# chao1224/GeoSSL

Measured on AMD Instinct MI355X. Metric: molecules/s/GPU SchNet+DDM fwd+bwd (QM9-sized, bs=1024); % HBM roofline, higher is better.
Workload: dtype f32

## Files before the change

### geossl_amd/csrc/ncsn_bwd.hip

```cpp
#include "common.h"
#include "geossl_hip.h"
#include "split.h"
#include "tn.h"

using namespace geossl;

namespace {

constexpr int TR = 32;

#ifdef NB_TIMING
__device__ long long nb_dbg[2 * 32 * 8];
#define NB_MARK(slot)                                                                              \
  do {                                                                                             \
    if (blockIdx.x == 5 && lane == 0 && (wave == 0 || wave == NW) && t - t_begin < 32)             \
      nb_dbg[((wave == 0 ? 0 : 1) * 32 + (t - t_begin)) * 8 + (slot)] = clock64();                 \
  } while (0)
#else
#define NB_MARK(slot) do {} while (0)
#endif

template <int NW>
struct NbLds {
  static constexpr int F = 32 * NW, H = F / 2, KHS = (H + 15) / 16, HMB = (H + 31) / 32, KS = F / 16;
  u32x4* zb;
  u32x4* dz2T;
  u32x4* fT;
  u32x4* dz1r;
  u32x4* abT;
  int4* scal;
  float* pdv;
  float* dep;
  float* wls;
  int* eg;
  int* ef;
  int* ea;
  int* ec;
  __device__ explicit NbLds(uint8_t* smem) {
    zb = reinterpret_cast<u32x4*>(smem);
    dz2T = zb + 2 * KHS * 2 * 64;
    fT = dz2T + HMB * 2 * 2 * 64;
    dz1r = fT + 2 * NW * 2 * 2 * 64;
    abT = dz1r + KS * 2 * 64;
    scal = reinterpret_cast<int4*>(abT + NW * 2 * 2 * 64);
    pdv = reinterpret_cast<float*>(scal + 3 * TR);
    dep = pdv + 3 * TR;
    wls = dep + NW * TR;
    eg = reinterpret_cast<int*>(wls + F);
    ef = eg + 4;
    ea = ef + 2 * NW;
    ec = ea + NW;
  }
  static size_t bytes() {
    return (size_t)(2 * KHS * 2 + HMB * 4 + 2 * NW * 4 + KS * 2 + NW * 4) * 1024 + 3 * TR * sizeof(int4) +
           (size_t)(3 * TR + NW * TR + F) * sizeof(float) + (size_t)(4 + 4 * NW) * sizeof(int);
  }
};

struct NcsnFusedArgs {
  const float* h;
  const int64_t* sei0;
  const int64_t* sei1;
  int S;
  GeosslNcsnWeights w;
  GeosslNcsnSaved sv;
  const int64_t* divisor;
  float out_scale;
  const float* gout;
  float* dfeat;
  float* demb;
  float* grow;
  float* pw1;
  float* pd1;
  float* pb1;
  float* pw2;
  float* pb2;
  float* psm;
};

__device__ __forceinline__ float ldg_off(const float* base, uint32_t byte_off) {
  return *reinterpret_cast<const float*>(reinterpret_cast<const char*>(base) + byte_off);
}
__device__ __forceinline__ int crow4(int r, int k4) { return (r & 3) + 8 * (r >> 2) + k4; }
__device__ __forceinline__ int opaque(int v) {
  asm volatile("" : "+v"(v));
  return v;
}
__device__ __forceinline__ u32x4 pack8(const f32x16& t, int s) {
  u32x4 w;
#pragma unroll
  for (int q = 0; q < 4; ++q) {
    const f16x2 p = {(_Float16)t[8 * s + 2 * q], (_Float16)t[8 * s + 2 * q + 1]};
    w[q] = __builtin_bit_cast(uint32_t, p);
  }
  return w;
}
__device__ __forceinline__ const u32x4& piece(const Frag2& f, int pc) { return pc == 0 ? f.h : f.l; }
__device__ __forceinline__ int scale_exponent(float m) { return max(mag_exponent(m), -40); }
__device__ __forceinline__ float pow2(int e) { return __builtin_amdgcn_ldexpf(1.0f, e); }
constexpr int E_NONE = -100000;

template <int NW, bool ROLE_A>
__device__ __forceinline__ void ncsn_bwd_body(const NcsnFusedArgs& a, const int S, const float* __restrict__ a_h) {
  using L_t = NbLds<NW>;
  constexpr int F = L_t::F, H = L_t::H, KHS = L_t::KHS, HMB = L_t::HMB, KS = L_t::KS, NT = 128 * NW;
  extern __shared__ __attribute__((aligned(16))) uint8_t smem_raw[];
  const L_t L(smem_raw);
  const int tid = threadIdx.x, lane = tid & 63, j = lane & 31, kh = lane >> 5;
  const int wave = __builtin_amdgcn_readfirstlane(tid >> 6);
  const int nb = ROLE_A ? wave : wave - NW;
  const int ntiles = (S + TR - 1) / TR;
  const int per = (ntiles + (int)gridDim.x - 1) / (int)gridDim.x;
  const int t_begin = (int)blockIdx.x * per, t_end = min(ntiles, t_begin + per);
  const float scale = a.out_scale * (a.gout != nullptr ? a.gout[0] : 1.0f) / (float)a.divisor[0];
  const uint32_t col = 32 * nb + j;

  Frag2 wreg[ROLE_A ? KHS : KS];
  f32x16 accw1[ROLE_A ? NW : 1];
  f32x16 accw2[ROLE_A ? 1 : HMB];
  int E1[ROLE_A ? NW : 1];
  int E2 = E_NONE;
  int ew = 0;
  float bsum = 0.0f, dsum = 0.0f;
  u32x4 ident[2];
  float w3r[8];
  float s_w2 = 0.0f, s_w1 = 0.0f, s_b1 = 0.0f, s_g = 0.0f, s_d = 0.0f;
  float iw1 = 0.0f, ib1 = 0.0f, iw2 = 0.0f;
  int e3;
  {
    float m3 = 0.0f;
    for (int i = lane; i < H; i += 64) m3 = fmaxf(m3, fabsf(a.w.o3_w[i]));
    e3 = scale_exponent(wave_max(m3));
  }
  if constexpr (ROLE_A) {
    iw1 = a.w.in_w1[col];
    ib1 = a.w.in_b1[col];
    iw2 = a.w.in_w2[col];
    float raw[KHS][8];
    float wm = 0.0f, csum = 0.0f;
#pragma unroll
    for (int ks = 0; ks < KHS; ++ks)
#pragma unroll
      for (int e = 0; e < 8; ++e) {
        const int m = 16 * ks + 8 * kh + e;
        const float v = m < H ? a.w.o2_w[(size_t)m * F + col] : 0.0f;
        raw[ks][e] = v;
        wm = fmaxf(wm, fabsf(v));
        csum = fmaf(fabsf(v), m < H ? fabsf(a.w.o3_w[m]) : 0.0f, csum);
      }
    ew = scale_exponent(wave_max(wm));
    const float sw = pow2(14 - ew);
#pragma unroll
    for (int ks = 0; ks < KHS; ++ks) wreg[ks] = split8h_scaled(raw[ks], sw);
    csum += __shfl_xor(csum, 32, 64);
    const int ecw = max(mag_exponent(wave_max(csum)), -80);
    if (lane == 0) L.ec[nb] = ecw;
#pragma unroll
    for (int kb = 0; kb < NW; ++kb) {
      E1[kb] = E_NONE;
#pragma unroll
      for (int r = 0; r < 16; ++r) accw1[kb][r] = 0.0f;
    }
#pragma unroll
    for (int s = 0; s < 2; ++s)
#pragma unroll
      for (int q = 0; q < 4; ++q) {
        const int k0 = 16 * s + kperm(2 * q, kh), k1 = 16 * s + kperm(2 * q + 1, kh);
        ident[s][q] = (k0 == j ? 0x3C00u : 0u) | (k1 == j ? 0x3C000000u : 0u);
      }
  } else {
    float raw[KS][8];
    float wm = 0.0f;
#pragma unroll
    for (int ks = 0; ks < KS; ++ks)
#pragma unroll
      for (int e = 0; e < 8; ++e) {
        raw[ks][e] = a.w.o1_w[(size_t)(16 * ks + kperm(e, kh)) * (F + 1) + col];
        wm = fmaxf(wm, fabsf(raw[ks][e]));
      }
    ew = scale_exponent(wave_max(wm));
    const float sw = pow2(14 - ew);
#pragma unroll
    for (int ks = 0; ks < KS; ++ks) wreg[ks] = split8h_scaled(raw[ks], sw);
#pragma unroll
    for (int e = 0; e < 8; ++e) {
      const int m = 16 * nb + 8 * kh + e;
      w3r[e] = (nb < KHS && m < H) ? a.w.o3_w[m] : 0.0f;
    }
#pragma unroll
    for (int mb = 0; mb < HMB; ++mb)
#pragma unroll
      for (int r = 0; r < 16; ++r) accw2[mb][r] = 0.0f;
#pragma unroll
    for (int q2 = 0; q2 < 2; ++q2)
#pragma unroll
      for (int q = 0; q < 4; ++q) {
        const int k0 = 16 * q2 + 8 * kh + 2 * q;
        ident[q2][q] = (k0 == j ? 0x3C00u : 0u) | (k0 + 1 == j ? 0x3C000000u : 0u);
      }
  }
  for (int i = tid; i < F; i += NT) L.wls[i] = a.w.o1_w[(size_t)i * (F + 1) + F];

  int sc_u = 0, sc_v = 0;
  float sc_g = 0.0f, sc_e = 0.0f, sc_p = 0.0f;
  int EG = -60;
  auto load_scal = [&](int tt) {
    if constexpr (ROLE_A) {
      if (wave == 0) {
        const int row = min(TR * tt + j, S - 1);
        sc_u = (int)a.sei0[row];
        sc_v = (int)a.sei1[row];
        sc_g = a.sv.gscale[row];
        sc_e = a.sv.emb[row];
        sc_p = a.sv.pd[row];
      }
    }
  };
  auto put_scal = [&](int tt) {
    if constexpr (ROLE_A) {
      if (wave == 0) {
        const int row = TR * tt + lane;
        const bool valid = lane < TR && row < S && tt < t_end;
        const float gr = valid ? pin(sc_g) * scale : 0.0f;
        EG = max(EG, mag_exponent(wave_max(fabsf(gr))));
        if (lane < TR) {
          L.scal[(tt % 3) * TR + lane] = make_int4(sc_u, sc_v, __float_as_int(gr), __float_as_int(sc_e));
          L.pdv[(tt % 3) * TR + lane] = sc_p;
          if (valid) a.grow[row] = gr;
        }
        if (lane == 0) L.eg[tt % 3] = EG;
      }
    }
  };
  float a1raw[16];
  auto request_a1 = [&](int tt, int k4) {
    if constexpr (ROLE_A) {
#pragma unroll
      for (int r = 0; r < 16; ++r)
        a1raw[r] = ldg_off(a.sv.a1, ((uint32_t)min(TR * tt + crow4(r, k4), S - 1) * (uint32_t)F + col) * 4u);
    }
  };
  f32x4 a2raw[2];
  float o3acc[8] = {0.0f, 0.0f, 0.0f, 0.0f, 0.0f, 0.0f, 0.0f, 0.0f};
  auto request_a2 = [&](int tt) {
    if constexpr (!ROLE_A) {
      if (nb < KHS) {
        const uint32_t off = ((uint32_t)min(TR * tt + j, S - 1) * (uint32_t)H + (16 * nb + 8 * kh)) * 4u;
        a2raw[0] = *reinterpret_cast<const f32x4*>(reinterpret_cast<const char*>(a.sv.a2) + off);
        a2raw[1] = *reinterpret_cast<const f32x4*>(reinterpret_cast<const char*>(a.sv.a2) + 16 + off);
      }
    }
  };
  float hu[16], hv[16];
  auto request_gather = [&](int tt, int k4) {
    if constexpr (!ROLE_A) {
      const int2* sc = reinterpret_cast<const int2*>(L.scal + (tt % 3) * TR);
#pragma unroll
      for (int r = 0; r < 16; ++r) {
        const int2 uv = sc[2 * crow4(r, k4)];
        hu[r] = ldg_off(a_h, ((uint32_t)uv.x * (uint32_t)F + col) * 4u);
        hv[r] = ldg_off(a_h, ((uint32_t)uv.y * (uint32_t)F + col) * 4u);
      }
    }
  };
  auto build_zb = [&](int tt) {
    if constexpr (!ROLE_A) {
      if (nb < KHS) {
        const float gr = __int_as_float(L.scal[(tt % 3) * TR + j].z);
        const float sz = pow2(14 - e3 - __builtin_amdgcn_readfirstlane(L.eg[tt % 3]));
        const float av[8] = {a2raw[0].x, a2raw[0].y, a2raw[0].z, a2raw[0].w, a2raw[1].x, a2raw[1].y, a2raw[1].z, a2raw[1].w};
        float v[8];
#pragma unroll
        for (int e = 0; e < 8; ++e) {
          const float a2v = pin(av[e]);
          v[e] = a2v > 0.0f ? gr * w3r[e] : 0.0f;
          o3acc[e] = fmaf(gr, a2v, o3acc[e]);
        }
        const Frag2 f = split8h_scaled(v, sz);
        u32x4* dst = L.zb + (size_t)(((tt & 1) * KHS + nb) * 2) * 64 + lane;
        dst[0] = f.h;
        dst[64] = f.l;
      }
    }
  };
  int EF = -40;
  auto build_fT = [&](int tt) {
    if constexpr (!ROLE_A) {
      float v[16];
      float m = 0.0f;
#pragma unroll
      for (int r = 0; r < 16; ++r) {
        v[r] = pin(hu[r]) + pin(hv[r]);
        m = fmaxf(m, fabsf(v[r]));
      }
      EF = max(EF, mag_exponent(wave_max(m)));
      const float sf = pow2(14 - EF);
      if (lane == 0) L.ef[(tt & 1) * NW + nb] = EF;
#pragma unroll
      for (int s = 0; s < 2; ++s) {
        float vv[8];
#pragma unroll
        for (int e = 0; e < 8; ++e) vv[e] = v[8 * s + e];
        const Frag2 f = split8h_scaled(vv, sf);
        u32x4* dst = L.fT + (size_t)((((tt & 1) * NW + nb) * 2 + s) * 2) * 64 + lane;
        dst[0] = f.h;
        dst[64] = f.l;
      }
    }
  };

  load_scal(t_begin);
  put_scal(t_begin);
  load_scal(t_begin + 1);
  put_scal(t_begin + 1);
  load_scal(t_begin + 2);
  if (t_begin < t_end) {
    request_a1(t_begin, 4 * kh);
    request_a2(t_begin);
  }
  __syncthreads();
  int eC = -80;
#pragma unroll
  for (int i = 0; i < NW; ++i) eC = max(eC, __builtin_amdgcn_readfirstlane(L.ec[i]));
  if (t_begin < t_end) {
    request_gather(t_begin, 4 * kh);
    build_zb(t_begin);
    build_fT(t_begin);
    request_a2(t_begin + 1);
    request_gather(t_begin + 1, 4 * kh);
  }
  int EA = -40;
  const float kA = pow2(e3 + ew - eC - 14);
  for (int t = t_begin; t < t_end; ++t) {
    const int buf = t & 1;
    int k4 = opaque(4 * kh);
    NB_MARK(0);
    lds_barrier();
    NB_MARK(1);
    const int EGt = __builtin_amdgcn_readfirstlane(L.eg[t % 3]);
    if constexpr (ROLE_A) {
      put_scal(t + 2);
      const float kT = pow2(EGt + eC - 14);
      f32x16 acc0, acc1;
#pragma unroll
      for (int r = 0; r < 16; ++r) acc0[r] = acc1[r] = 0.0f;
      {
        const u32x4* zs = L.zb + (size_t)(buf * KHS * 2) * 64 + lane;
        Frag2 a0, an;
        a0.h = zs[0]; a0.l = zs[64];
#pragma unroll
        for (int ks = 0; ks < KHS; ++ks) {
          if (ks + 1 < KHS) {
            const u32x4* s0 = zs + (size_t)((ks + 1) * 2) * 64;
            an.h = s0[0]; an.l = s0[64];
          }
          __builtin_amdgcn_sched_barrier(0);
          mma3x2(acc0, acc1, a0, wreg[ks]);
          __builtin_amdgcn_sched_barrier(0);
          if (ks + 1 < KHS) a0 = an;
        }
      }
      NB_MARK(5);
      float v[16];
      {
        const int4* sc = L.scal + (t % 3) * TR;
        float tb = 0.0f, td = 0.0f, am = 0.0f;
#pragma unroll
        for (int r = 0; r < 16; ++r) {
          a1raw[r] = pin(a1raw[r]);
          v[r] = a1raw[r] > 0.0f ? (acc0[r] + acc1[r]) * kA : 0.0f;
          tb += v[r];
          td = fmaf(v[r], __int_as_float(sc[crow4(r, k4)].w), td);
          am = fmaxf(am, fabsf(a1raw[r]));
        }
        bsum = fmaf(tb, kT, bsum);
        dsum = fmaf(td, kT, dsum);
        EA = max(EA, mag_exponent(wave_max(am)));
      }
      {
        const float sa = pow2(14 - EA);
        if (lane == 0) L.ea[nb] = EA;
#pragma unroll
        for (int s = 0; s < 2; ++s) {
          float vv[8];
#pragma unroll
          for (int e = 0; e < 8; ++e) vv[e] = a1raw[8 * s + e];
          const Frag2 f = split8h_scaled(vv, sa);
          u32x4* dst = L.abT + (size_t)((nb * 2 + s) * 2) * 64 + lane;
          dst[0] = f.h;
          dst[64] = f.l;
        }
      }
      Frag2 da[2];
#pragma unroll
      for (int s = 0; s < 2; ++s) {
        float vv[8];
#pragma unroll
        for (int e = 0; e < 8; ++e) vv[e] = v[8 * s + e];
        da[s] = split8h(vv);
      }
      {
        float wl[16];
#pragma unroll
        for (int r = 0; r < 16; ++r) wl[r] = L.wls[32 * nb + crow4(r, k4)];
        float de = 0.0f;
#pragma unroll
        for (int pc = 1; pc >= 0; --pc) {
          f32x16 tp;
#pragma unroll
          for (int r = 0; r < 16; ++r) tp[r] = 0.0f;
          tp = mfma_f16(piece(da[0], pc), ident[0], tp);
          tp = mfma_f16(piece(da[1], pc), ident[1], tp);
#pragma unroll
          for (int r = 0; r < 16; ++r) de = fmaf(tp[r], wl[r], de);
#pragma unroll
          for (int half = 0; half < 2; ++half)
            L.dz1r[(size_t)((2 * nb + half) * 2 + pc) * 64 + lane] = pack8(tp, half);
        }
        de += __shfl_xor(de, 32, 64);
        if (kh == 0) L.dep[j * NW + nb] = de * kT;
      }
      NB_MARK(6);
#pragma unroll
      for (int kb = 0; kb < NW; ++kb) {
        const int En = EGt + __builtin_amdgcn_readfirstlane(L.ef[buf * NW + kb]);
        if (En != E1[kb]) {
          const float f = pow2(max(E1[kb] - En, -200));
#pragma unroll
          for (int r = 0; r < 16; ++r) accw1[kb][r] *= f;
          E1[kb] = En;
        }
#pragma unroll
        for (int s = 0; s < 2; ++s) {
          const u32x4* s0 = L.fT + (size_t)(((buf * NW + kb) * 2 + s) * 2) * 64 + lane;
          Frag2 bf;
          bf.h = s0[0]; bf.l = s0[64];
          mma3(accw1[kb], da[s], bf);
        }
      }
    } else {
      if (nb < HMB) {
        float tb = 0.0f;
#pragma unroll
        for (int pc = 1; pc >= 0; --pc) {
          f32x16 tp;
#pragma unroll
          for (int r = 0; r < 16; ++r) tp[r] = 0.0f;
#pragma unroll
          for (int q = 0; q < 2; ++q) {
            if (2 * nb + q < KHS) {
              const u32x4* s0 = L.zb + (size_t)((buf * KHS + 2 * nb + q) * 2 + pc) * 64 + lane;
              tp = mfma_f16(s0[0], ident[q], tp);
            }
          }
#pragma unroll
          for (int r = 0; r < 16; ++r) tb += tp[r];
#pragma unroll
          for (int s = 0; s < 2; ++s) L.dz2T[(size_t)((nb * 2 + s) * 2 + pc) * 64 + lane] = pack8(tp, s);
        }
        bsum = fmaf(tb, pow2(EGt + e3 - 14), bsum);
      }
      NB_MARK(5);
      build_zb(t + 1);
      NB_MARK(6);
      build_fT(t + 1);
    }
    k4 = opaque(4 * kh);
    NB_MARK(2);
    lds_barrier();
    NB_MARK(3);
    if constexpr (ROLE_A) {
      request_a1(t + 1, k4);
      load_scal(t + 3);
      {
        const int4* sc = L.scal + (t % 3) * TR;
        const float* pdr = L.pdv + (t % 3) * TR;
#pragma unroll
        for (int i = 0; i < 16; ++i) {
          const int rl = 4 * k4 + i;
          float de = 0.0f;
#pragma unroll
          for (int n2 = 0; n2 < NW; ++n2) de += L.dep[rl * NW + n2];
          const float pd = pdr[rl];
          const float pre = fmaf(iw1, pd, ib1);
          s_w2 = fmaf(de, fmaxf(pre, 0.0f), s_w2);
          const float dp = pre > 0.0f ? de * iw2 : 0.0f;
          s_w1 = fmaf(dp, pd, s_w1);
          s_b1 += dp;
          if (wave == 0 && j == i) {
            s_g += __int_as_float(sc[rl].z);
            s_d += de;
          }
        }
      }
    } else {
      request_a2(t + 2);
      request_gather(t + 2, k4);
      NB_MARK(7);
      f32x16 acc0, acc1;
#pragma unroll
      for (int r = 0; r < 16; ++r) acc0[r] = acc1[r] = 0.0f;
      {
        const u32x4* zs = L.dz1r + lane;
        Frag2 b0, bn;
        b0.h = zs[0]; b0.l = zs[64];
#pragma unroll
        for (int ks = 0; ks < KS; ++ks) {
          if (ks + 1 < KS) {
            const u32x4* s0 = zs + (size_t)((ks + 1) * 2) * 64;
            bn.h = s0[0]; bn.l = s0[64];
          }
          __builtin_amdgcn_sched_barrier(0);
          mma3x2(acc0, acc1, wreg[ks], b0);
          __builtin_amdgcn_sched_barrier(0);
          if (ks + 1 < KS) b0 = bn;
        }
      }
      const float kD = pow2(EGt + eC + ew - 28);
      f32x16 outp;
#pragma unroll
      for (int r = 0; r < 16; ++r) outp[r] = (acc0[r] + acc1[r]) * kD;
      const int row = TR * t + j;
      if (row < S) {
        const uint32_t off = ((uint32_t)row * (uint32_t)F + 32 * nb + 4 * kh) * 4u;
#pragma unroll
        for (int q = 0; q < 4; ++q)
          *reinterpret_cast<f32x4*>(reinterpret_cast<char*>(a.dfeat) + 32 * q + off) =
              f32x4{outp[4 * q], outp[4 * q + 1], outp[4 * q + 2], outp[4 * q + 3]};
        if (nb == 0 && kh == 0) {
          float de = 0.0f;
#pragma unroll
          for (int n2 = 0; n2 < NW; ++n2) de += L.dep[j * NW + n2];
          a.demb[row] = de;
        }
      }
      {
        const int En = EGt + __builtin_amdgcn_readfirstlane(L.ea[nb]);
        if (En != E2) {
          const float f = pow2(max(E2 - En, -200));
#pragma unroll
          for (int mb = 0; mb < HMB; ++mb)
#pragma unroll
            for (int r = 0; r < 16; ++r) accw2[mb][r] *= f;
          E2 = En;
        }
      }
#pragma unroll
      for (int s = 0; s < 2; ++s) {
        const u32x4* sb = L.abT + (size_t)((nb * 2 + s) * 2) * 64 + lane;
        Frag2 bf;
        bf.h = sb[0]; bf.l = sb[64];
#pragma unroll
        for (int mb = 0; mb < HMB; ++mb) {
          const u32x4* s0 = L.dz2T + (size_t)((mb * 2 + s) * 2) * 64 + lane;
          Frag2 af;
          af.h = s0[0]; af.l = s0[64];
          mma3(accw2[mb], af, bf);
        }
      }
    }
    NB_MARK(4);
  }
  const size_t pb = blockIdx.x;
  if constexpr (ROLE_A) {
    float* P1 = a.pw1 + pb * F * F;
#pragma unroll
    for (int kb = 0; kb < NW; ++kb) {
      const float f = pow2(max(E1[kb] + eC - 28, -200));
#pragma unroll
      for (int r = 0; r < 16; ++r) P1[(size_t)(32 * nb + c_row(r, lane)) * F + 32 * kb + j] = accw1[kb][r] * f;
    }
    const float sb = bsum + __shfl_xor(bsum, 32, 64), sd = dsum + __shfl_xor(dsum, 32, 64);
    if (kh == 0) {
      a.pb1[pb * F + col] = sb;
      a.pd1[pb * F + col] = sd;
    }
    float* Ps = a.psm + pb * (H + 3 * F + 2);
    const float t_w2 = s_w2 + __shfl_xor(s_w2, 32, 64);
    const float t_w1 = s_w1 + __shfl_xor(s_w1, 32, 64), t_b1 = s_b1 + __shfl_xor(s_b1, 32, 64);
    if (kh == 0) {
      Ps[H + col] = t_w2;
      Ps[H + F + col] = t_w1;
      Ps[H + 2 * F + col] = t_b1;
    }
    if (wave == 0) {
      const float tg = wave_sum(s_g), td = wave_sum(s_d);
      if (lane == 0) {
        Ps[H + 3 * F] = tg;
        Ps[H + 3 * F + 1] = td;
      }
    }
  } else {
    float* P2 = a.pw2 + pb * H * F;
    const float f = pow2(max(E2 + e3 - 28, -200));
#pragma unroll
    for (int mb = 0; mb < HMB; ++mb)
#pragma unroll
      for (int r = 0; r < 16; ++r) {
        const int m = 32 * mb + c_row(r, lane);
        if (m < H) P2[(size_t)m * F + col] = accw2[mb][r] * f;
      }
    const float sb = bsum + __shfl_xor(bsum, 32, 64);
    if (nb < HMB && kh == 0 && (int)col < H) a.pb2[pb * H + col] = sb;
    if (nb < KHS) {
      float* Ps = a.psm + pb * (H + 3 * F + 2);
#pragma unroll
      for (int e = 0; e < 8; ++e) {
        float v = o3acc[e];
#pragma unroll
        for (int o = 16; o > 0; o >>= 1) v += __shfl_xor(v, o, 64);
        const int m = 16 * nb + 8 * kh + e;
        if (j == 0 && m < H) Ps[m] = v;
      }
    }
  }
}

template <int NW>
__global__ __launch_bounds__(128 * NW) void k_ncsn_bwd_fused(NcsnFusedArgs a) {
  if ((int)(threadIdx.x >> 6) < NW) ncsn_bwd_body<NW, true>(a, a.S, a.h);
  else ncsn_bwd_body<NW, false>(a, a.S, a.h);
}
struct NcsnFusedPair { NcsnFusedArgs a[2]; };
template <int NW>
__global__ __launch_bounds__(128 * NW) void k_ncsn_bwd_fused2(NcsnFusedPair pr, const int32_t* __restrict__ dyn_S,
                                                              const int32_t* __restrict__ dyn_view) {
  const NcsnFusedArgs& a = pr.a[blockIdx.y];
  const int S = dyn_count(a.S, dyn_S);
  const float* h = a.h;
  if (dyn_view != nullptr && blockIdx.y == 1) h += (size_t)(*dyn_view) * (32 * NW);
  if ((int)(threadIdx.x >> 6) < NW) ncsn_bwd_body<NW, true>(a, S, h);
  else ncsn_bwd_body<NW, false>(a, S, h);
}

__device__ __forceinline__ void ncsn_reduce_all_block(const ReduceMulti& m, int nblk, int accumulate,
                                                      const float* __restrict__ psm, int F, const GeosslNcsnGrads& g,
                                                      float (*red)[64]) {
  const int mb = m.xoff[m.nseg];
  if ((int)blockIdx.x < mb) {
    reduce_multi_block(m, nblk, accumulate, red, 0);
    return;
  }
  const int H = F / 2, len = H + 3 * F + 2;
  const int i = ((int)blockIdx.x - mb) * 4 + (int)(threadIdx.x >> 6), lane = threadIdx.x & 63;
  if (i >= len) return;
  float s = 0.0f;
  for (int b = lane; b < nblk; b += 64) s += psm[(size_t)b * len + i];
  s = wave_sum(s);
  if (lane == 0) {
    float* dst;
    if (i < H) dst = g.o3_w + i;
    else if (i < H + F) dst = g.in_w2 + (i - H);
    else if (i < H + 2 * F) dst = g.in_w1 + (i - H - F);
    else if (i < H + 3 * F) dst = g.in_b1 + (i - H - 2 * F);
    else if (i == H + 3 * F) dst = g.o3_b;
    else dst = g.in_b2;
    *dst = accumulate ? *dst + s : s;
  }
}
__global__ __launch_bounds__(256) void k_ncsn_reduce_all(ReduceMulti m, int nblk, int accumulate,
                                                         const float* __restrict__ psm, int F, GeosslNcsnGrads g) {
  __shared__ float red[4][64];
  ncsn_reduce_all_block(m, nblk, accumulate, psm, F, g, red);
}
__global__ __launch_bounds__(256) void k_ncsn_reduce_all2(ReduceMulti m0, ReduceMulti m1, int nblk, int accumulate,
                                                          const float* __restrict__ psm0,
                                                          const float* __restrict__ psm1, int F, GeosslNcsnGrads g0,
                                                          GeosslNcsnGrads g1) {
  __shared__ float red[4][64];
  if (blockIdx.y == 0) ncsn_reduce_all_block(m0, nblk, accumulate, psm0, F, g0, red);
  else ncsn_reduce_all_block(m1, nblk, accumulate, psm1, F, g1, red);
}

inline int fused_blocks(int64_t S) {
  const int64_t ntiles = (S + TR - 1) / TR;
  return (int)(ntiles < 256 ? ntiles : 256);
}

}

#ifdef NB_TIMING
extern "C" int geossl_ncsn_bwd_debug_read(long long* host) {
  return (int)hipMemcpyFromSymbol(host, HIP_SYMBOL(nb_dbg), sizeof(long long) * 2 * 32 * 8);
}
#endif

extern "C" int64_t geossl_ddm_loss_bwd_fused_workspace_floats(int64_t S, int F) {
  const int64_t nb = fused_blocks(S), H = F / 2;
  return nb * ((int64_t)F * F + 2 * F + H * F + H + (H + 3 * F + 2));
}

extern "C" int geossl_ddm_loss_bwd_fused(const float* h, const int64_t* sei0, const int64_t* sei1, int64_t S, int64_t N,
                                         int F, const GeosslNcsnWeights* w, const GeosslNcsnSaved* saved,
                                         const int64_t* stats_divisor, float out_scale, const float* gout, float* dfeat,
                                         float* demb, float* grow, const GeosslNcsnGrads* grads, float* workspace,
                                         int accumulate, hipStream_t stream) {
  if (S <= 0) return 0;
  if (F != 32 && F != 64 && F != 128) return (int)hipErrorInvalidValue;
  if (S * (int64_t)F * 4 >= ((int64_t)1 << 32) || N * (int64_t)F * 4 >= ((int64_t)1 << 32)) return (int)hipErrorInvalidValue;
  const int nb = fused_blocks(S), H = F / 2;
  NcsnFusedArgs a;
  a.h = h; a.sei0 = sei0; a.sei1 = sei1; a.S = (int)S; a.w = *w; a.sv = *saved; a.divisor = stats_divisor;
  a.out_scale = out_scale; a.gout = gout; a.dfeat = dfeat; a.demb = demb; a.grow = grow;
  a.pw1 = workspace;
  a.pd1 = a.pw1 + (size_t)nb * F * F;
  a.pb1 = a.pd1 + (size_t)nb * F;
  a.pw2 = a.pb1 + (size_t)nb * F;
  a.pb2 = a.pw2 + (size_t)nb * H * F;
  a.psm = a.pb2 + (size_t)nb * H;
#define LAUNCH(NWV)                                                                                      \
  do {                                                                                                   \
    allow_big_lds(&k_ncsn_bwd_fused<NWV>);                                                               \
    hipLaunchKernelGGL((k_ncsn_bwd_fused<NWV>), dim3(nb), dim3(128 * NWV), NbLds<NWV>::bytes(), stream, a); \
  } while (0)
  if (F == 128) LAUNCH(4); else if (F == 64) LAUNCH(2); else LAUNCH(1);
#undef LAUNCH
  GEOSSL_CHECK_LAUNCH();
  ReduceMulti rm;
  float* o1w[1] = {grads->o1_w};
  float* o1c[1] = {grads->o1_w + F};
  float* o1b[1] = {grads->o1_b};
  float* o2w[1] = {grads->o2_w};
  float* o2b[1] = {grads->o2_b};
  rm.add(a.pw1, F * F, F, F + 1, 1, o1w, 1);
  rm.add(a.pd1, F, F, F, F + 1, o1c, 1);
  rm.add(a.pb1, F, F, F, 1, o1b, 1);
  rm.add(a.pw2, H * F, F, F, 1, o2w, 1);
  rm.add(a.pb2, H, H, H, 1, o2b, 1);
  hipLaunchKernelGGL(k_ncsn_reduce_all, dim3(rm.blocks() + (H + 3 * F + 2 + 3) / 4, 1), dim3(256), 0, stream, rm, nb,
                     accumulate, a.psm, F, *grads);
  GEOSSL_CHECK_LAUNCH();
  return 0;
}

namespace geossl {
int launch_incidence_gather2(const float* dfeat0, const float* dfeat1, const int64_t* inc_ptr, const int32_t* inc_idx,
                             int64_t N, int F, float* dh0, float* dh1, hipStream_t stream, const int32_t* dyn_view);
}

extern "C" int geossl_ddm_loss_bwd_fused2(const GeosslNcsnHeadBwd* heads, const int64_t* sei0, const int64_t* sei1,
                                          int64_t S, int64_t N, int F, const int64_t* stats_divisor, const float* gout,
                                          const int64_t* inc_ptr, const int32_t* inc_idx, int accumulate,
                                          hipStream_t stream) {
  return geossl_ddm_loss_bwd_fused2_dyn(heads, sei0, sei1, S, N, F, stats_divisor, gout, inc_ptr, inc_idx, accumulate,
                                        nullptr, nullptr, stream);
}

extern "C" int geossl_ddm_loss_bwd_fused2_dyn(const GeosslNcsnHeadBwd* heads, const int64_t* sei0, const int64_t* sei1,
                                              int64_t S, int64_t N, int F, const int64_t* stats_divisor,
                                              const float* gout, const int64_t* inc_ptr, const int32_t* inc_idx,
                                              int accumulate, const int32_t* dyn_S, const int32_t* dyn_view,
                                              hipStream_t stream) {
  if (S <= 0) return 0;
  if (heads == nullptr || (F != 32 && F != 64 && F != 128)) return (int)hipErrorInvalidValue;
  if (S * (int64_t)F * 4 >= ((int64_t)1 << 32) || N * (int64_t)F * 4 >= ((int64_t)1 << 32)) return (int)hipErrorInvalidValue;
  const int nb = (fused_blocks(S) + 1) / 2, H = F / 2;
  NcsnFusedPair pr;
  NcsnFusedArgs* a = pr.a;
  for (int k = 0; k < 2; ++k) {
    const GeosslNcsnHeadBwd& hd = heads[k];
    if (hd.h == nullptr || hd.dfeat == nullptr || hd.workspace == nullptr) return (int)hipErrorInvalidValue;
    NcsnFusedArgs& x = a[k];
    x.h = hd.h; x.sei0 = sei0; x.sei1 = sei1; x.S = (int)S; x.w = hd.w; x.sv = hd.saved; x.divisor = stats_divisor;
    x.out_scale = hd.out_scale; x.gout = gout; x.dfeat = hd.dfeat; x.demb = hd.demb; x.grow = hd.grow;
    x.pw1 = hd.workspace;
    x.pd1 = x.pw1 + (size_t)nb * F * F;
    x.pb1 = x.pd1 + (size_t)nb * F;
    x.pw2 = x.pb1 + (size_t)nb * F;
    x.pb2 = x.pw2 + (size_t)nb * H * F;
    x.psm = x.pb2 + (size_t)nb * H;
  }
#define LAUNCH2(NWV)                                                                                                \
  do {                                                                                                              \
    allow_big_lds(&k_ncsn_bwd_fused2<NWV>);                                                                         \
    hipLaunchKernelGGL((k_ncsn_bwd_fused2<NWV>), dim3(nb, 2), dim3(128 * NWV), NbLds<NWV>::bytes(), stream, pr,         \
                       dyn_S, dyn_view);                                                                            \
  } while (0)
  if (F == 128) LAUNCH2(4); else if (F == 64) LAUNCH2(2); else LAUNCH2(1);
#undef LAUNCH2
  GEOSSL_CHECK_LAUNCH();
  ReduceMulti rm[2];
  for (int k = 0; k < 2; ++k) {
    const GeosslNcsnGrads* grads = &heads[k].grads;
    float* o1w[1] = {grads->o1_w};
    float* o1c[1] = {grads->o1_w + F};
    float* o1b[1] = {grads->o1_b};
    float* o2w[1] = {grads->o2_w};
    float* o2b[1] = {grads->o2_b};
    rm[k].add(a[k].pw1, F * F, F, F + 1, 1, o1w, 1);
    rm[k].add(a[k].pd1, F, F, F, F + 1, o1c, 1);
    rm[k].add(a[k].pb1, F, F, F, 1, o1b, 1);
    rm[k].add(a[k].pw2, H * F, F, F, 1, o2w, 1);
    rm[k].add(a[k].pb2, H, H, H, 1, o2b, 1);
  }
  hipLaunchKernelGGL(k_ncsn_reduce_all2, dim3(rm[0].blocks() + (H + 3 * F + 2 + 3) / 4, 2), dim3(256), 0, stream, rm[0],
                     rm[1], nb, accumulate, a[0].psm, a[1].psm, F, heads[0].grads, heads[1].grads);
  GEOSSL_CHECK_LAUNCH();
  if (heads[0].dh != nullptr && heads[1].dh != nullptr)
    return launch_incidence_gather2(heads[0].dfeat, heads[1].dfeat, inc_ptr, inc_idx, N, F, heads[0].dh, heads[1].dh, stream,
                                    dyn_view);
  return 0;
}
```

Measured before the change: 430,100.

## Process two 32-row sub-tiles per barrier in fused NCSN backward kernel

Doubles the per-iteration row tile in the fused NCSN backward kernel to 64 rows, handled as two 32-row sub-tiles. Each LDS barrier now covers twice the work, and the a1/a2/gather prefetches are restructured around the sub-tiles. Several per-lane weight registers (o3_w, in_w1/b1/w2) move into LDS, and waves_per_eu(2) is added, both to ease register pressure. The old 32-row path stays available through an environment variable. The cost is more LDS per block, and the grid still uses the 32-row block count, so fewer tiles per block may hurt load balance.

```diff
diff --git a/geossl_amd/csrc/ncsn_bwd.hip b/geossl_amd/csrc/ncsn_bwd.hip
--- a/geossl_amd/csrc/ncsn_bwd.hip
+++ b/geossl_amd/csrc/ncsn_bwd.hip
@@ -19,10 +19,16 @@
 #else
 #define NB_MARK(slot) do {} while (0)
 #endif
-
-template <int NW>
+#ifdef NB_HALF_BARRIERS
+#define NB_TILE_BARRIER() do { if (((t - t_begin) & 1) == 0) lds_barrier(); } while (0)
+#else
+#define NB_TILE_BARRIER() lds_barrier()
+#endif
+
+template <int NW, int MB>
 struct NbLds {
   static constexpr int F = 32 * NW, H = F / 2, KHS = (H + 15) / 16, HMB = (H + 31) / 32, KS = F / 16;
+  static constexpr int TT = TR * MB, FB = MB == 1 ? 2 : 1;
   u32x4* zb;
   u32x4* dz2T;
   u32x4* fT;
@@ -32,28 +38,33 @@
   float* pdv;
   float* dep;
   float* wls;
+  float* w3s;
+  float* inw;
   int* eg;
   int* ef;
   int* ea;
   int* ec;
   __device__ explicit NbLds(uint8_t* smem) {
     zb = reinterpret_cast<u32x4*>(smem);
-    dz2T = zb + 2 * KHS * 2 * 64;
-    fT = dz2T + HMB * 2 * 2 * 64;
-    dz1r = fT + 2 * NW * 2 * 2 * 64;
-    abT = dz1r + KS * 2 * 64;
-    scal = reinterpret_cast<int4*>(abT + NW * 2 * 2 * 64);
-    pdv = reinterpret_cast<float*>(scal + 3 * TR);
-    dep = pdv + 3 * TR;
-    wls = dep + NW * TR;
-    eg = reinterpret_cast<int*>(wls + F);
-    ef = eg + 4;
-    ea = ef + 2 * NW;
-    ec = ea + NW;
+    dz2T = zb + 2 * MB * KHS * 2 * 64;
+    fT = dz2T + MB * HMB * 2 * 2 * 64;
+    dz1r = fT + FB * MB * NW * 2 * 2 * 64;
+    abT = dz1r + MB * KS * 2 * 64;
+    scal = reinterpret_cast<int4*>(abT + MB * NW * 2 * 2 * 64);
+    pdv = reinterpret_cast<float*>(scal + 3 * TT);
+    dep = pdv + 3 * TT;
+    wls = dep + NW * TT;
+    w3s = wls + F;
+    inw = w3s + 16 * KHS;
+    eg = reinterpret_cast<int*>(inw + 3 * F);
+    ef = eg + 8;
+    ea = ef + FB * MB * NW;
+    ec = ea + MB * NW;
   }
   static size_t bytes() {
-    return (size_t)(2 * KHS * 2 + HMB * 4 + 2 * NW * 4 + KS * 2 + NW * 4) * 1024 + 3 * TR * sizeof(int4) +
-           (size_t)(3 * TR + NW * TR + F) * sizeof(float) + (size_t)(4 + 4 * NW) * sizeof(int);
+    return (size_t)(MB * (2 * KHS * 2 + HMB * 4 + FB * NW * 4 + KS * 2 + NW * 4)) * 1024 + 3 * TT * sizeof(int4) +
+           (size_t)(3 * TT + NW * TT + F + 16 * KHS + 3 * F) * sizeof(float) +
+           (size_t)(8 + FB * MB * NW + MB * NW + NW) * sizeof(int);
   }
 };
 
@@ -76,6 +87,7 @@
   float* pw2;
   float* pb2;
   float* psm;
+  int tile32;
 };
 
 __device__ __forceinline__ float ldg_off(const float* base, uint32_t byte_off) {
@@ -100,16 +112,18 @@
 __device__ __forceinline__ float pow2(int e) { return __builtin_amdgcn_ldexpf(1.0f, e); }
 constexpr int E_NONE = -100000;
 
-template <int NW, bool ROLE_A>
+template <int NW, bool ROLE_A, int MB>
 __device__ __forceinline__ void ncsn_bwd_body(const NcsnFusedArgs& a, const int S, const float* __restrict__ a_h) {
-  using L_t = NbLds<NW>;
+  using L_t = NbLds<NW, MB>;
   constexpr int F = L_t::F, H = L_t::H, KHS = L_t::KHS, HMB = L_t::HMB, KS = L_t::KS, NT = 128 * NW;
+  constexpr int TT = L_t::TT;
+  constexpr bool FT2 = MB == 2;
   extern __shared__ __attribute__((aligned(16))) uint8_t smem_raw[];
   const L_t L(smem_raw);
   const int tid = threadIdx.x, lane = tid & 63, j = lane & 31, kh = lane >> 5;
   const int wave = __builtin_amdgcn_readfirstlane(tid >> 6);
   const int nb = ROLE_A ? wave : wave - NW;
-  const int ntiles = (S + TR - 1) / TR;
+  const int ntiles = (S + TT - 1) / TT;
   const int per = (ntiles + (int)gridDim.x - 1) / (int)gridDim.x;
   const int t_begin = (int)blockIdx.x * per, t_end = min(ntiles, t_begin + per);
   const float scale = a.out_scale * (a.gout != nullptr ? a.gout[0] : 1.0f) / (float)a.divisor[0];
@@ -123,9 +137,7 @@
   int ew = 0;
   float bsum = 0.0f, dsum = 0.0f;
   u32x4 ident[2];
-  float w3r[8];
   float s_w2 = 0.0f, s_w1 = 0.0f, s_b1 = 0.0f, s_g = 0.0f, s_d = 0.0f;
-  float iw1 = 0.0f, ib1 = 0.0f, iw2 = 0.0f;
   int e3;
   {
     float m3 = 0.0f;
@@ -133,9 +145,6 @@
     e3 = scale_exponent(wave_max(m3));
   }
   if constexpr (ROLE_A) {
-    iw1 = a.w.in_w1[col];
-    ib1 = a.w.in_b1[col];
-    iw2 = a.w.in_w2[col];
     float raw[KHS][8];
     float wm = 0.0f, csum = 0.0f;
 #pragma unroll
@@ -183,11 +192,6 @@
 #pragma unroll
     for (int ks = 0; ks < KS; ++ks) wreg[ks] = split8h_scaled(raw[ks], sw);
 #pragma unroll
-    for (int e = 0; e < 8; ++e) {
-      const int m = 16 * nb + 8 * kh + e;
-      w3r[e] = (nb < KHS && m < H) ? a.w.o3_w[m] : 0.0f;
-    }
-#pragma unroll
     for (int mb = 0; mb < HMB; ++mb)
 #pragma unroll
       for (int r = 0; r < 16; ++r) accw2[mb][r] = 0.0f;
@@ -199,7 +203,13 @@
         ident[q2][q] = (k0 == j ? 0x3C00u : 0u) | (k0 + 1 == j ? 0x3C000000u : 0u);
       }
   }
-  for (int i = tid; i < F; i += NT) L.wls[i] = a.w.o1_w[(size_t)i * (F + 1) + F];
+  for (int i = tid; i < F; i += NT) {
+    L.wls[i] = a.w.o1_w[(size_t)i * (F + 1) + F];
+    L.inw[i] = a.w.in_w1[i];
+    L.inw[F + i] = a.w.in_b1[i];
+    L.inw[2 * F + i] = a.w.in_w2[i];
+  }
+  for (int i = tid; i < 16 * KHS; i += NT) L.w3s[i] = i < H ? a.w.o3_w[i] : 0.0f;
 
   int sc_u = 0, sc_v = 0;
   float sc_g = 0.0f, sc_e = 0.0f, sc_p = 0.0f;
@@ -207,7 +217,7 @@
   auto load_scal = [&](int tt) {
     if constexpr (ROLE_A) {
       if (wave == 0) {
-        const int row = min(TR * tt + j, S - 1);
+        const int row = min(TT * tt + (lane & (TT - 1)), S - 1);
         sc_u = (int)a.sei0[row];
         sc_v = (int)a.sei1[row];
         sc_g = a.sv.gscale[row];
@@ -219,42 +229,54 @@
   auto put_scal = [&](int tt) {
     if constexpr (ROLE_A) {
       if (wave == 0) {
-        const int row = TR * tt + lane;
-        const bool valid = lane < TR && row < S && tt < t_end;
+        const int row = TT * tt + lane;
+        const bool valid = lane < TT && row < S && tt < t_end;
         const float gr = valid ? pin(sc_g) * scale : 0.0f;
-        EG = max(EG, mag_exponent(wave_max(fabsf(gr))));
-        if (lane < TR) {
-          L.scal[(tt % 3) * TR + lane] = make_int4(sc_u, sc_v, __float_as_int(gr), __float_as_int(sc_e));
-          L.pdv[(tt % 3) * TR + lane] = sc_p;
+        if constexpr (MB == 1) {
+          EG = max(EG, mag_exponent(wave_max(fabsf(gr))));
+          if (lane == 0) L.eg[tt % 3] = EG;
+        } else {
+          float m = fabsf(gr);
+#pragma unroll
+          for (int o = 16; o > 0; o >>= 1) m = fmaxf(m, __shfl_xor(m, o, 64));
+          const int e0 = max(EG, mag_exponent(__int_as_float(__builtin_amdgcn_readlane(__float_as_int(m), 0))));
+          EG = max(e0, mag_exponent(__int_as_float(__builtin_amdgcn_readlane(__float_as_int(m), 32))));
+          if (lane == 0) {
+            L.eg[(tt % 3) * MB] = e0;
+            L.eg[(tt % 3) * MB + 1] = EG;
+          }
+        }
+        if (lane < TT) {
+          L.scal[(tt % 3) * TT + lane] = make_int4(sc_u, sc_v, __float_as_int(gr), __float_as_int(sc_e));
+          L.pdv[(tt % 3) * TT + lane] = sc_p;
           if (valid) a.grow[row] = gr;
         }
-        if (lane == 0) L.eg[tt % 3] = EG;
       }
     }
   };
   float a1raw[16];
-  auto request_a1 = [&](int tt, int k4) {
+  auto request_a1 = [&](int tt, int sb, int k4) {
     if constexpr (ROLE_A) {
 #pragma unroll
       for (int r = 0; r < 16; ++r)
-        a1raw[r] = ldg_off(a.sv.a1, ((uint32_t)min(TR * tt + crow4(r, k4), S - 1) * (uint32_t)F + col) * 4u);
+        a1raw[r] = ldg_off(a.sv.a1, ((uint32_t)min(TT * tt + TR * sb + crow4(r, k4), S - 1) * (uint32_t)F + col) * 4u);
     }
   };
-  f32x4 a2raw[2];
+  f32x4 a2raw[MB][2];
   float o3acc[8] = {0.0f, 0.0f, 0.0f, 0.0f, 0.0f, 0.0f, 0.0f, 0.0f};
-  auto request_a2 = [&](int tt) {
+  auto request_a2 = [&](int tt, int sb) {
     if constexpr (!ROLE_A) {
       if (nb < KHS) {
-        const uint32_t off = ((uint32_t)min(TR * tt + j, S - 1) * (uint32_t)H + (16 * nb + 8 * kh)) * 4u;
-        a2raw[0] = *reinterpret_cast<const f32x4*>(reinterpret_cast<const char*>(a.sv.a2) + off);
-        a2raw[1] = *reinterpret_cast<const f32x4*>(reinterpret_cast<const char*>(a.sv.a2) + 16 + off);
+        const uint32_t off = ((uint32_t)min(TT * tt + TR * sb + j, S - 1) * (uint32_t)H + (16 * nb + 8 * kh)) * 4u;
+        a2raw[sb][0] = *reinterpret_cast<const f32x4*>(reinterpret_cast<const char*>(a.sv.a2) + off);
+        a2raw[sb][1] = *reinterpret_cast<const f32x4*>(reinterpret_cast<const char*>(a.sv.a2) + 16 + off);
       }
     }
   };
   float hu[16], hv[16];
-  auto request_gather = [&](int tt, int k4) {
+  auto request_gather = [&](int tt, int sb, int k4) {
     if constexpr (!ROLE_A) {
-      const int2* sc = reinterpret_cast<const int2*>(L.scal + (tt % 3) * TR);
+      const int2* sc = reinterpret_cast<const int2*>(L.scal + (tt % 3) * TT + TR * sb);
 #pragma unroll
       for (int r = 0; r < 16; ++r) {
         const int2 uv = sc[2 * crow4(r, k4)];
@@ -263,12 +285,16 @@
       }
     }
   };
-  auto build_zb = [&](int tt) {
+  auto build_zb = [&](int tt, int sb) {
     if constexpr (!ROLE_A) {
       if (nb < KHS) {
-        const float gr = __int_as_float(L.scal[(tt % 3) * TR + j].z);
-        const float sz = pow2(14 - e3 - __builtin_amdgcn_readfirstlane(L.eg[tt % 3]));
-        const float av[8] = {a2raw[0].x, a2raw[0].y, a2raw[0].z, a2raw[0].w, a2raw[1].x, a2raw[1].y, a2raw[1].z, a2raw[1].w};
+        const float gr = __int_as_float(L.scal[(tt % 3) * TT + TR * sb + j].z);
+        const float sz = pow2(14 - e3 - __builtin_amdgcn_readfirstlane(L.eg[(tt % 3) * MB + sb]));
+        const f32x4 q0 = a2raw[sb][0], q1 = a2raw[sb][1];
+        const f32x4 w0 = *reinterpret_cast<const f32x4*>(L.w3s + 16 * nb + 8 * kh);
+        const f32x4 w1 = *reinterpret_cast<const f32x4*>(L.w3s + 16 * nb + 8 * kh + 4);
+        const float w3r[8] = {w0.x, w0.y, w0.z, w0.w, w1.x, w1.y, w1.z, w1.w};
+        const float av[8] = {q0.x, q0.y, q0.z, q0.w, q1.x, q1.y, q1.z, q1.w};
         float v[8];
 #pragma unroll
         for (int e = 0; e < 8; ++e) {
@@ -277,14 +303,14 @@
           o3acc[e] = fmaf(gr, a2v, o3acc[e]);
         }
         const Frag2 f = split8h_scaled(v, sz);
-        u32x4* dst = L.zb + (size_t)(((tt & 1) * KHS + nb) * 2) * 64 + lane;
+        u32x4* dst = L.zb + (size_t)(((((tt & 1) * MB + sb) * KHS) + nb) * 2) * 64 + lane;
         dst[0] = f.h;
         dst[64] = f.l;
       }
     }
   };
   int EF = -40;
-  auto build_fT = [&](int tt) {
+  auto build_fT = [&](int tt, int sb) {
     if constexpr (!ROLE_A) {
       float v[16];
       float m = 0.0f;
@@ -295,14 +321,15 @@
       }
       EF = max(EF, mag_exponent(wave_max(m)));
       const float sf = pow2(14 - EF);
-      if (lane == 0) L.ef[(tt & 1) * NW + nb] = EF;
+      const int fb = FT2 ? 0 : (tt & 1);
+      if (lane == 0) L.ef[(fb * MB + sb) * NW + nb] = EF;
 #pragma unroll
       for (int s = 0; s < 2; ++s) {
         float vv[8];
 #pragma unroll
         for (int e = 0; e < 8; ++e) vv[e] = v[8 * s + e];
         const Frag2 f = split8h_scaled(vv, sf);
-        u32x4* dst = L.fT + (size_t)((((tt & 1) * NW + nb) * 2 + s) * 2) * 64 + lane;
+        u32x4* dst = L.fT + (size_t)(((((fb * MB + sb) * NW) + nb) * 2 + s) * 2) * 64 + lane;
         dst[0] = f.h;
         dst[64] = f.l;
       }
@@ -315,19 +342,23 @@
   put_scal(t_begin + 1);
   load_scal(t_begin + 2);
   if (t_begin < t_end) {
-    request_a1(t_begin, 4 * kh);
-    request_a2(t_begin);
+    request_a1(t_begin, 0, 4 * kh);
+#pragma unroll
+    for (int sb = 0; sb < MB; ++sb) request_a2(t_begin, sb);
   }
   __syncthreads();
   int eC = -80;
 #pragma unroll
   for (int i = 0; i < NW; ++i) eC = max(eC, __builtin_amdgcn_readfirstlane(L.ec[i]));
   if (t_begin < t_end) {
-    request_gather(t_begin, 4 * kh);
-    build_zb(t_begin);
-    build_fT(t_begin);
-    request_a2(t_begin + 1);
-    request_gather(t_begin + 1, 4 * kh);
+    request_gather(t_begin, 0, 4 * kh);
+#pragma unroll
+    for (int sb = 0; sb < MB; ++sb) build_zb(t_begin, sb);
+    build_fT(t_begin, 0);
+#pragma unroll
+    for (int sb = 0; sb < MB; ++sb) request_a2(t_begin + 1, sb);
+    if constexpr (FT2) request_gather(t_begin, 1, 4 * kh);
+    else request_gather(t_begin + 1, 0, 4 * kh);
   }
   int EA = -40;
   const float kA = pow2(e3 + ew - eC - 14);
@@ -335,152 +366,177 @@
     const int buf = t & 1;
     int k4 = opaque(4 * kh);
     NB_MARK(0);
-    lds_barrier();
+    NB_TILE_BARRIER();
     NB_MARK(1);
-    const int EGt = __builtin_amdgcn_readfirstlane(L.eg[t % 3]);
+    auto EGof = [&](int sb) { return __builtin_amdgcn_readfirstlane(L.eg[(t % 3) * MB + sb]); };
+    Frag2 da[2];
+    auto dw1 = [&](int sb) {
+      if constexpr (ROLE_A) {
+        const int fb = FT2 ? 0 : buf;
+#pragma unroll
+        for (int kb = 0; kb < NW; ++kb) {
+          const int En = EGof(sb) + __builtin_amdgcn_readfirstlane(L.ef[(fb * MB + sb) * NW + kb]);
+          if (En != E1[kb]) {
+            const float f = pow2(max(E1[kb] - En, -200));
+#pragma unroll
+            for (int r = 0; r < 16; ++r) accw1[kb][r] *= f;
+            E1[kb] = En;
+          }
+#pragma unroll
+          for (int s = 0; s < 2; ++s) {
+            const u32x4* s0 = L.fT + (size_t)(((((fb * MB + sb) * NW) + kb) * 2 + s) * 2) * 64 + lane;
+            Frag2 bf;
+            bf.h = s0[0]; bf.l = s0[64];
+            mma3(accw1[kb], da[s], bf);
+          }
+        }
+      }
+    };
     if constexpr (ROLE_A) {
       put_scal(t + 2);
-      const float kT = pow2(EGt + eC - 14);
-      f32x16 acc0, acc1;
-#pragma unroll
-      for (int r = 0; r < 16; ++r) acc0[r] = acc1[r] = 0.0f;
-      {
-        const u32x4* zs = L.zb + (size_t)(buf * KHS * 2) * 64 + lane;
-        Frag2 a0, an;
-        a0.h = zs[0]; a0.l = zs[64];
-#pragma unroll
-        for (int ks = 0; ks < KHS; ++ks) {
-          if (ks + 1 < KHS) {
-            const u32x4* s0 = zs + (size_t)((ks + 1) * 2) * 64;
-            an.h = s0[0]; an.l = s0[64];
-          }
-          __builtin_amdgcn_sched_barrier(0);
-          mma3x2(acc0, acc1, a0, wreg[ks]);
-          __builtin_amdgcn_sched_barrier(0);
-          if (ks + 1 < KHS) a0 = an;
-        }
-      }
-      NB_MARK(5);
-      float v[16];
-      {
-        const int4* sc = L.scal + (t % 3) * TR;
-        float tb = 0.0f, td = 0.0f, am = 0.0f;
-#pragma unroll
-        for (int r = 0; r < 16; ++r) {
-          a1raw[r] = pin(a1raw[r]);
-          v[r] = a1raw[r] > 0.0f ? (acc0[r] + acc1[r]) * kA : 0.0f;
-          tb += v[r];
-          td = fmaf(v[r], __int_as_float(sc[crow4(r, k4)].w), td);
-          am = fmaxf(am, fabsf(a1raw[r]));
-        }
-        bsum = fmaf(tb, kT, bsum);
-        dsum = fmaf(td, kT, dsum);
-        EA = max(EA, mag_exponent(wave_max(am)));
-      }
-      {
-        const float sa = pow2(14 - EA);
-        if (lane == 0) L.ea[nb] = EA;
+#pragma unroll 1
+      for (int sb = 0; sb < MB; ++sb) {
+        if (sb > 0) k4 = opaque(4 * kh);
+        const float kT = pow2(EGof(sb) + eC - 14);
+        f32x16 acc0, acc1;
+#pragma unroll
+        for (int r = 0; r < 16; ++r) acc0[r] = acc1[r] = 0.0f;
+        {
+          const u32x4* zs = L.zb + (size_t)((buf * MB + sb) * KHS * 2) * 64 + lane;
+          Frag2 a0, an;
+          a0.h = zs[0]; a0.l = zs[64];
+#pragma unroll
+          for (int ks = 0; ks < KHS; ++ks) {
+            if (ks + 1 < KHS) {
+              const u32x4* s0 = zs + (size_t)((ks + 1) * 2) * 64;
+              an.h = s0[0]; an.l = s0[64];
+            }
+            __builtin_amdgcn_sched_barrier(0);
+            mma3x2(acc0, acc1, a0, wreg[ks]);
+            __builtin_amdgcn_sched_barrier(0);
+            if (ks + 1 < KHS) a0 = an;
+          }
+        }
+        if (sb == 0) NB_MARK(5);
+        float v[16];
+        {
+          const int4* sc = L.scal + (t % 3) * TT + TR * sb;
+          float tb = 0.0f, td = 0.0f, am = 0.0f;
+#pragma unroll
+          for (int r = 0; r < 16; ++r) {
+            a1raw[r] = pin(a1raw[r]);
+            v[r] = a1raw[r] > 0.0f ? (acc0[r] + acc1[r]) * kA : 0.0f;
+            tb += v[r];
+            td = fmaf(v[r], __int_as_float(sc[crow4(r, k4)].w), td);
+            am = fmaxf(am, fabsf(a1raw[r]));
+          }
+          bsum = fmaf(tb, kT, bsum);
+          dsum = fmaf(td, kT, dsum);
+          EA = max(EA, mag_exponent(wave_max(am)));
+        }
+        {
+          const float sa = pow2(14 - EA);
+          if (lane == 0) L.ea[sb * NW + nb] = EA;
+#pragma unroll
+          for (int s = 0; s < 2; ++s) {
+            float vv[8];
+#pragma unroll
+            for (int e = 0; e < 8; ++e) vv[e] = a1raw[8 * s + e];
+            const Frag2 f = split8h_scaled(vv, sa);
+            u32x4* dst = L.abT + (size_t)(((sb * NW + nb) * 2 + s) * 2) * 64 + lane;
+            dst[0] = f.h;
+            dst[64] = f.l;
+          }
+        }
+        if constexpr (MB == 2) request_a1(sb == 0 ? t : t + 1, sb == 0 ? 1 : 0, k4);
 #pragma unroll
         for (int s = 0; s < 2; ++s) {
           float vv[8];
 #pragma unroll
-          for (int e = 0; e < 8; ++e) vv[e] = a1raw[8 * s + e];
-          const Frag2 f = split8h_scaled(vv, sa);
-          u32x4* dst = L.abT + (size_t)((nb * 2 + s) * 2) * 64 + lane;
-          dst[0] = f.h;
-          dst[64] = f.l;
-        }
-      }
-      Frag2 da[2];
-#pragma unroll
-      for (int s = 0; s < 2; ++s) {
-        float vv[8];
-#pragma unroll
-        for (int e = 0; e < 8; ++e) vv[e] = v[8 * s + e];
-        da[s] = split8h(vv);
-      }
-      {
-        float wl[16];
-#pragma unroll
-        for (int r = 0; r < 16; ++r) wl[r] = L.wls[32 * nb + crow4(r, k4)];
-        float de = 0.0f;
-#pragma unroll
-        for (int pc = 1; pc >= 0; --pc) {
-          f32x16 tp;
-#pragma unroll
-          for (int r = 0; r < 16; ++r) tp[r] = 0.0f;
-          tp = mfma_f16(piece(da[0], pc), ident[0], tp);
-          tp = mfma_f16(piece(da[1], pc), ident[1], tp);
-#pragma unroll
-          for (int r = 0; r < 16; ++r) de = fmaf(tp[r], wl[r], de);
-#pragma unroll
-          for (int half = 0; half < 2; ++half)
-            L.dz1r[(size_t)((2 * nb + half) * 2 + pc) * 64 + lane] = pack8(tp, half);
-        }
-        de += __shfl_xor(de, 32, 64);
-        if (kh == 0) L.dep[j * NW + nb] = de * kT;
-      }
-      NB_MARK(6);
-#pragma unroll
-      for (int kb = 0; kb < NW; ++kb) {
-        const int En = EGt + __builtin_amdgcn_readfirstlane(L.ef[buf * NW + kb]);
-        if (En != E1[kb]) {
-          const float f = pow2(max(E1[kb] - En, -200));
-#pragma unroll
-          for (int r = 0; r < 16; ++r) accw1[kb][r] *= f;
-          E1[kb] = En;
-        }
-#pragma unroll
-        for (int s = 0; s < 2; ++s) {
-          const u32x4* s0 = L.fT + (size_t)(((buf * NW + kb) * 2 + s) * 2) * 64 + lane;
-          Frag2 bf;
-          bf.h = s0[0]; bf.l = s0[64];
-          mma3(accw1[kb], da[s], bf);
-        }
+          for (int e = 0; e < 8; ++e) vv[e] = v[8 * s + e];
+          da[s] = split8h(vv);
+        }
+        {
+          float wl[16];
+#pragma unroll
+          for (int r = 0; r < 16; ++r) wl[r] = L.wls[32 * nb + crow4(r, k4)];
+          float de = 0.0f;
+#pragma unroll
+          for (int pc = 1; pc >= 0; --pc) {
+            f32x16 tp;
+#pragma unroll
+            for (int r = 0; r < 16; ++r) tp[r] = 0.0f;
+            tp = mfma_f16(piece(da[0], pc), ident[0], tp);
+            tp = mfma_f16(piece(da[1], pc), ident[1], tp);
+#pragma unroll
+            for (int r = 0; r < 16; ++r) de = fmaf(tp[r], wl[r], de);
+#pragma unroll
+            for (int half = 0; half < 2; ++half)
+              L.dz1r[(size_t)((sb * KS + 2 * nb + half) * 2 + pc) * 64 + lane] = pack8(tp, half);
+          }
+          de += __shfl_xor(de, 32, 64);
+          if (kh == 0) L.dep[(TR * sb + j) * NW + nb] = de * kT;
+        }
+        if (sb == 0) NB_MARK(6);
+        if (!FT2 || sb == 0) dw1(sb);
       }
     } else {
       if (nb < HMB) {
-        float tb = 0.0f;
-#pragma unroll
-        for (int pc = 1; pc >= 0; --pc) {
-          f32x16 tp;
-#pragma unroll
-          for (int r = 0; r < 16; ++r) tp[r] = 0.0f;
-#pragma unroll
-          for (int q = 0; q < 2; ++q) {
-            if (2 * nb + q < KHS) {
-              const u32x4* s0 = L.zb + (size_t)((buf * KHS + 2 * nb + q) * 2 + pc) * 64 + lane;
-              tp = mfma_f16(s0[0], ident[q], tp);
+#pragma unroll
+        for (int sb = 0; sb < MB; ++sb) {
+          float tb = 0.0f;
+#pragma unroll
+          for (int pc = 1; pc >= 0; --pc) {
+            f32x16 tp;
+#pragma unroll
+            for (int r = 0; r < 16; ++r) tp[r] = 0.0f;
+#pragma unroll
+            for (int q = 0; q < 2; ++q) {
+              if (2 * nb + q < KHS) {
+                const u32x4* s0 = L.zb + (size_t)(((buf * MB + sb) * KHS + 2 * nb + q) * 2 + pc) * 64 + lane;
+                tp = mfma_f16(s0[0], ident[q], tp);
+              }
             }
-          }
-#pragma unroll
-          for (int r = 0; r < 16; ++r) tb += tp[r];
-#pragma unroll
-          for (int s = 0; s < 2; ++s) L.dz2T[(size_t)((nb * 2 + s) * 2 + pc) * 64 + lane] = pack8(tp, s);
-        }
-        bsum = fmaf(tb, pow2(EGt + e3 - 14), bsum);
+#pragma unroll
+            for (int r = 0; r < 16; ++r) tb += tp[r];
+#pragma unroll
+            for (int s = 0; s < 2; ++s)
+              L.dz2T[(size_t)(((sb * HMB + nb) * 2 + s) * 2 + pc) * 64 + lane] = pack8(tp, s);
+          }
+          bsum = fmaf(tb, pow2(EGof(sb) + e3 - 14), bsum);
+        }
       }
       NB_MARK(5);
-      build_zb(t + 1);
+#pragma unroll
+      for (int sb = 0; sb < MB; ++sb) build_zb(t + 1, sb);
       NB_MARK(6);
-      build_fT(t + 1);
+      if constexpr (FT2) build_fT(t, 1);
+      else build_fT(t + 1, 0);
     }
     k4 = opaque(4 * kh);
     NB_MARK(2);
-    lds_barrier();
+    NB_TILE_BARRIER();
     NB_MARK(3);
     if constexpr (ROLE_A) {
-      request_a1(t + 1, k4);
+      if constexpr (MB == 1) request_a1(t + 1, 0, k4);
       load_scal(t + 3);
-      {
-        const int4* sc = L.scal + (t % 3) * TR;
-        const float* pdr = L.pdv + (t % 3) * TR;
+      if constexpr (FT2) {
+        dw1(1);
+        __builtin_amdgcn_sched_barrier(0);
+      }
+#pragma unroll 1
+      for (int sb = 0; sb < MB; ++sb) {
+        const int4* sc = L.scal + (t % 3) * TT + TR * sb;
+        const float* pdr = L.pdv + (t % 3) * TT + TR * sb;
+        const float* dpr = L.dep + TR * sb * NW;
+        const float iw1 = L.inw[col], ib1 = L.inw[F + col], iw2 = L.inw[2 * F + col];
+        if (sb > 0) k4 = opaque(4 * kh);
 #pragma unroll
         for (int i = 0; i < 16; ++i) {
           const int rl = 4 * k4 + i;
           float de = 0.0f;
 #pragma unroll
-          for (int n2 = 0; n2 < NW; ++n2) de += L.dep[rl * NW + n2];
+          for (int n2 = 0; n2 < NW; ++n2) de += dpr[rl * NW + n2];
           const float pd = pdr[rl];
           const float pre = fmaf(iw1, pd, ib1);
           s_w2 = fmaf(de, fmaxf(pre, 0.0f), s_w2);
@@ -494,69 +550,86 @@
         }
       }
     } else {
-      request_a2(t + 2);
-      request_gather(t + 2, k4);
+      if constexpr (!FT2) request_a2(t + 2, 0);
+      request_gather(FT2 ? t + 1 : t + 2, 0, k4);
       NB_MARK(7);
-      f32x16 acc0, acc1;
-#pragma unroll
-      for (int r = 0; r < 16; ++r) acc0[r] = acc1[r] = 0.0f;
-      {
-        const u32x4* zs = L.dz1r + lane;
-        Frag2 b0, bn;
-        b0.h = zs[0]; b0.l = zs[64];
-#pragma unroll
-        for (int ks = 0; ks < KS; ++ks) {
-          if (ks + 1 < KS) {
-            const u32x4* s0 = zs + (size_t)((ks + 1) * 2) * 64;
-            bn.h = s0[0]; bn.l = s0[64];
-          }
-          __builtin_amdgcn_sched_barrier(0);
-          mma3x2(acc0, acc1, wreg[ks], b0);
-          __builtin_amdgcn_sched_barrier(0);
-          if (ks + 1 < KS) b0 = bn;
-        }
-      }
-      const float kD = pow2(EGt + eC + ew - 28);
-      f32x16 outp;
-#pragma unroll
-      for (int r = 0; r < 16; ++r) outp[r] = (acc0[r] + acc1[r]) * kD;
-      const int row = TR * t + j;
-      if (row < S) {
-        const uint32_t off = ((uint32_t)row * (uint32_t)F + 32 * nb + 4 * kh) * 4u;
-#pragma unroll
-        for (int q = 0; q < 4; ++q)
-          *reinterpret_cast<f32x4*>(reinterpret_cast<char*>(a.dfeat) + 32 * q + off) =
-              f32x4{outp[4 * q], outp[4 * q + 1], outp[4 * q + 2], outp[4 * q + 3]};
-        if (nb == 0 && kh == 0) {
-          float de = 0.0f;
-#pragma unroll
-          for (int n2 = 0; n2 < NW; ++n2) de += L.dep[j * NW + n2];
-          a.demb[row] = de;
-        }
-      }
-      {
-        const int En = EGt + __builtin_amdgcn_readfirstlane(L.ea[nb]);
-        if (En != E2) {
-          const float f = pow2(max(E2 - En, -200));
-#pragma unroll
-          for (int mb = 0; mb < HMB; ++mb)
-#pragma unroll
-            for (int r = 0; r < 16; ++r) accw2[mb][r] *= f;
-          E2 = En;
-        }
-      }
-#pragma unroll
-      for (int s = 0; s < 2; ++s) {
-        const u32x4* sb = L.abT + (size_t)((nb * 2 + s) * 2) * 64 + lane;
-        Frag2 bf;
-        bf.h = sb[0]; bf.l = sb[64];
-#pragma unroll
-        for (int mb = 0; mb < HMB; ++mb) {
-          const u32x4* s0 = L.dz2T + (size_t)((mb * 2 + s) * 2) * 64 + lane;
-          Frag2 af;
-          af.h = s0[0]; af.l = s0[64];
-          mma3(accw2[mb], af, bf);
-        }
+#pragma unroll 1
+      for (int sb = 0; sb < MB; ++sb) {
+        __builtin_amdgcn_sched_barrier(0);
+        f32x16 acc0, acc1;
+#pragma unroll
+        for (int r = 0; r < 16; ++r) acc0[r] = acc1[r] = 0.0f;
+        {
+          const u32x4* zs = L.dz1r + (size_t)(sb * KS * 2) * 64 + lane;
+          Frag2 b0, bn;
+          b0.h = zs[0]; b0.l = zs[64];
+#pragma unroll
+          for (int ks = 0; ks < KS; ++ks) {
+            if (ks + 1 < KS) {
+              const u32x4* s0 = zs + (size_t)((ks + 1) * 2) * 64;
+              bn.h = s0[0]; bn.l = s0[64];
+            }
+            __builtin_amdgcn_sched_barrier(0);
+            mma3x2(acc0, acc1, wreg[ks], b0);
+            __builtin_amdgcn_sched_barrier(0);
+            if (ks + 1 < KS) b0 = bn;
+          }
+        }
+        const float kD = pow2(EGof(sb) + eC + ew - 28);
+        f32x16 outp;
+#pragma unroll
+        for (int r = 0; r < 16; ++r) outp[r] = (acc0[r] + acc1[r]) * kD;
+        const int row = TT * t + TR * sb + j;
+        if (row < S) {
+          const uint32_t off = ((uint32_t)row * (uint32_t)F + 32 * nb + 4 * kh) * 4u;
+#pragma unroll
+          for (int q = 0; q < 4; ++q)
+            *reinterpret_cast<f32x4*>(reinterpret_cast<char*>(a.dfeat) + 32 * q + off) =
+                f32x4{outp[4 * q], outp[4 * q + 1], outp[4 * q + 2], outp[4 * q + 3]};
+          if (nb == 0 && kh == 0) {
+            float de = 0.0f;
+#pragma unroll
+            for (int n2 = 0; n2 < NW; ++n2) de += L.dep[(TR * sb + j) * NW + n2];
+            a.demb[row] = de;
+          }
+        }
+      }
+#pragma unroll 1
+      for (int sb = 0; sb < MB; ++sb) {
+        __builtin_amdgcn_sched_barrier(0);
+        {
+          const int En = EGof(sb) + __builtin_amdgcn_readfirstlane(L.ea[sb * NW + nb]);
+          if (En != E2) {
+            const float f = pow2(max(E2 - En, -200));
+#pragma unroll
+            for (int mb = 0; mb < HMB; ++mb)
+#pragma unroll
+              for (int r = 0; r < 16; ++r) accw2[mb][r] *= f;
+            E2 = En;
+          }
+        }
+#pragma unroll
+        for (int s = 0; s < 2; ++s) {
+          const u32x4* sa = L.abT + (size_t)(((sb * NW + nb) * 2 + s) * 2) * 64 + lane;
+          Frag2 bf;
+          bf.h = sa[0]; bf.l = sa[64];
+#pragma unroll
+          for (int mb = 0; mb < HMB; ++mb) {
+            const u32x4* s0 = L.dz2T + (size_t)(((sb * HMB + mb) * 2 + s) * 2) * 64 + lane;
+            Frag2 af;
+            af.h = s0[0]; af.l = s0[64];
+            mma3(accw2[mb], af, bf);
+          }
+        }
+      }
+      if constexpr (FT2) {
+        __builtin_amdgcn_sched_barrier(0);
+        build_fT(t + 1, 0);
+        k4 = opaque(4 * kh);
+        request_gather(t + 1, 1, k4);
+        __builtin_amdgcn_sched_barrier(0);
+#pragma unroll
+        for (int sb = 0; sb < MB; ++sb) request_a2(t + 2, sb);
       }
     }
     NB_MARK(4);
@@ -617,20 +690,28 @@
 }
 
 template <int NW>
-__global__ __launch_bounds__(128 * NW) void k_ncsn_bwd_fused(NcsnFusedArgs a) {
-  if ((int)(threadIdx.x >> 6) < NW) ncsn_bwd_body<NW, true>(a, a.S, a.h);
-  else ncsn_bwd_body<NW, false>(a, a.S, a.h);
+__device__ __forceinline__ void ncsn_bwd_roles(const NcsnFusedArgs& a, const int S, const float* __restrict__ h) {
+  if (a.tile32) {
+    if ((int)(threadIdx.x >> 6) < NW) ncsn_bwd_body<NW, true, 1>(a, S, h);
+    else ncsn_bwd_body<NW, false, 1>(a, S, h);
+  } else {
+    if ((int)(threadIdx.x >> 6) < NW) ncsn_bwd_body<NW, true, 2>(a, S, h);
+    else ncsn_bwd_body<NW, false, 2>(a, S, h);
+  }
+}
+template <int NW>
+__global__ __launch_bounds__(128 * NW) __attribute__((amdgpu_waves_per_eu(2))) void k_ncsn_bwd_fused(NcsnFusedArgs a) {
+  ncsn_bwd_roles<NW>(a, a.S, a.h);
 }
 struct NcsnFusedPair { NcsnFusedArgs a[2]; };
 template <int NW>
-__global__ __launch_bounds__(128 * NW) void k_ncsn_bwd_fused2(NcsnFusedPair pr, const int32_t* __restrict__ dyn_S,
-                                                              const int32_t* __restrict__ dyn_view) {
+__global__ __launch_bounds__(128 * NW) __attribute__((amdgpu_waves_per_eu(2))) void k_ncsn_bwd_fused2(
+    NcsnFusedPair pr, const int32_t* __restrict__ dyn_S, const int32_t* __restrict__ dyn_view) {
   const NcsnFusedArgs& a = pr.a[blockIdx.y];
   const int S = dyn_count(a.S, dyn_S);
   const float* h = a.h;
   if (dyn_view != nullptr && blockIdx.y == 1) h += (size_t)(*dyn_view) * (32 * NW);
-  if ((int)(threadIdx.x >> 6) < NW) ncsn_bwd_body<NW, true>(a, S, h);
-  else ncsn_bwd_body<NW, false>(a, S, h);
+  ncsn_bwd_roles<NW>(a, S, h);
 }
 
 __device__ __forceinline__ void ncsn_reduce_all_block(const ReduceMulti& m, int nblk, int accumulate,
@@ -676,6 +757,9 @@
   const int64_t ntiles = (S + TR - 1) / TR;
   return (int)(ntiles < 256 ? ntiles : 256);
 }
+inline int tile32_requested() { return getenv("GEOSSL_NCSN_BWD_TILE32") != nullptr ? 1 : 0; }
+template <int NW>
+inline size_t fused_lds_bytes(int tile32) { return tile32 ? NbLds<NW, 1>::bytes() : NbLds<NW, 2>::bytes(); }
 
 }
 
@@ -708,10 +792,12 @@
   a.pw2 = a.pb1 + (size_t)nb * F;
   a.pb2 = a.pw2 + (size_t)nb * H * F;
   a.psm = a.pb2 + (size_t)nb * H;
+  a.tile32 = tile32_requested();
 #define LAUNCH(NWV)                                                                                      \
   do {                                                                                                   \
     allow_big_lds(&k_ncsn_bwd_fused<NWV>);                                                               \
-    hipLaunchKernelGGL((k_ncsn_bwd_fused<NWV>), dim3(nb), dim3(128 * NWV), NbLds<NWV>::bytes(), stream, a); \
+    hipLaunchKernelGGL((k_ncsn_bwd_fused<NWV>), dim3(nb), dim3(128 * NWV), fused_lds_bytes<NWV>(a.tile32), stream, \
+                       a);                                                                               \
   } while (0)
   if (F == 128) LAUNCH(4); else if (F == 64) LAUNCH(2); else LAUNCH(1);
 #undef LAUNCH
@@ -755,6 +841,7 @@
   if (heads == nullptr || (F != 32 && F != 64 && F != 128)) return (int)hipErrorInvalidValue;
   if (S * (int64_t)F * 4 >= ((int64_t)1 << 32) || N * (int64_t)F * 4 >= ((int64_t)1 << 32)) return (int)hipErrorInvalidValue;
   const int nb = (fused_blocks(S) + 1) / 2, H = F / 2;
+  const int tile32 = tile32_requested();
   NcsnFusedPair pr;
   NcsnFusedArgs* a = pr.a;
   for (int k = 0; k < 2; ++k) {
@@ -769,12 +856,13 @@
     x.pw2 = x.pb1 + (size_t)nb * F;
     x.pb2 = x.pw2 + (size_t)nb * H * F;
     x.psm = x.pb2 + (size_t)nb * H;
+    x.tile32 = tile32;
   }
 #define LAUNCH2(NWV)                                                                                                \
   do {                                                                                                              \
     allow_big_lds(&k_ncsn_bwd_fused2<NWV>);                                                                         \
-    hipLaunchKernelGGL((k_ncsn_bwd_fused2<NWV>), dim3(nb, 2), dim3(128 * NWV), NbLds<NWV>::bytes(), stream, pr,         \
-                       dyn_S, dyn_view);                                                                            \
+    hipLaunchKernelGGL((k_ncsn_bwd_fused2<NWV>), dim3(nb, 2), dim3(128 * NWV), fused_lds_bytes<NWV>(tile32), stream, \
+                       pr, dyn_S, dyn_view);                                                                        \
   } while (0)
   if (F == 128) LAUNCH2(4); else if (F == 64) LAUNCH2(2); else LAUNCH2(1);
 #undef LAUNCH2
```

New measurement: 432,600 (median of 6 runs). Within noise of the previous version (+0.6%).
